# Sachin-A/TraceWeaver

Hardware: AMD Instinct MI355X
Metric: spans/sec reconstructed + assignment accuracy vs ground truth (higher is better)
Workload: dtype int64 timestamps, f64 scores; 1 GPU; media_microservices shape (6 services, E in {1,1,1,1,2,4}), 100000 requests/service x 16 replicas per GPU, concurrency 1.6, two-pass reconstruction, device mixture refit; spans_per_gpu=25600000, spans_total=25600000, parallelism=units sharded, 1 rank(s), backend none

## Files before the change

### traceweaver_amd/csrc/tw_engine.hip

```cpp
#include <algorithm>
#include <chrono>
#include <cmath>
#include <cstdio>
#include <cstdlib>
#include <cstring>
#include <functional>
#include <string>
#include <type_traits>
#include <vector>

#include <hip/hip_runtime.h>
#include <rocprim/rocprim.hpp>

#include "traceweaver_amd.h"
#include "tw_kernels.h"
#include "tw_fit.h"
#include "tw_eval.h"
#include "tw_skip.h"
#include "tw_load.h"
#include "tw_baselines.h"
#include "tw_stitch.h"
#include "tw_attr.h"
#include "tw_conf.h"
#include "tw_dist.h"
// ... 58 lines not shown
    hipEvent_t tile_ev[kMaxEp + 1] = {};
    hipStream_t cls_stream2[kMaxEp + 1] = {};
    hipEvent_t stretch_ev[kMaxEp + 1][kEnumStretches] = {}, stretch_done[kMaxEp + 1] = {};
    int enum_stretches = 1, stretch_min_tiles = 2048;
    int heavy_grid = 4096, select_grid = 0;
    int debug_lists = 0;
    int32_t first_lists[3][kMaxEp + 1] = {};
    hipEvent_t gate_ev = nullptr;
    int tile_gate = 0;
    int stage_min_tiles = 1024;
    int32_t *rank_in = nullptr, *rank_out = nullptr;
    bool class_params = false;
    int prio_min_e = 0, prio_high = 0;
    bool prio_any = false;
    int pipeline = 1;
    std::string err;
    int state = ST_EMPTY;
    int tile = kTile;
    int tile_threads = 2;
    int tile_single = 1;
    int tile_rank = 1;
    int block_params = 1;
    int tile_single_threads = 1;
    int coop = kCoop;
    std::vector<UnitDev> units;
    std::vector<TileDev> tiles;
    std::vector<int64_t> gs_off_h;
    std::vector<void*> allocs;
    void* arena = nullptr;
    size_t arena_cap = 0;
    bool arena_open = false;
    std::vector<std::pair<std::function<void(void*)>, size_t>> arena_req;
    Dev P{};
    int64_t n_ie = 0, n_gp = 0, n_slots = 0, n_gaps = 0;
    PairVI* agg_pair = nullptr;
    int32_t *agg_i32 = nullptr, *agg_i32b = nullptr;
    uint32_t *seg_in = nullptr, *seg_out = nullptr;
    int n_seg_out = 0;
    void* sort_tmp = nullptr;
    size_t sort_tmp_bytes = 0;
    double* mix_p_dev = nullptr;
    int32_t* mix_n_dev = nullptr;
    double* mix_c_dev = nullptr;
    double* gaps_sorted = nullptr;
    double* fit_models = nullptr;
    double* fit_uval = nullptr;
// ... 304 lines not shown
    const dim3 hb(std::min(e->coop, kHeavyThreads));
    const int pool = E > 4 ? 2048 : (E > 1 ? kPairPoolPerEp * E : 1);
    const size_t pool_bytes = sizeof(double) * (size_t)pool;
    const size_t lean_bytes = sizeof(double) * (size_t)(2 * kMaxEp * kNarrow + e->lean_pool), lean_bytes_w = sizeof(double) * (size_t)(2 * kMaxEp * 64 * kCandWords + e->lean_pool);
    const bool lean = E >= P.lean_min_e && !e->skip_mode;
    const int cap = P.heavy_in_off[E + 1] - P.heavy_in_off[E];
    auto grid_for = [&](int known, int most) { return std::max(std::min(((known >= 0 ? known : cap) + kWorkChunk - 1) / kWorkChunk, most), 1); };
    auto narrow = [&](int part, int g) {
        if (lean) hipLaunchKernelGGL((k_enumerate_lean<kNarrow>), dim3(g), hb, lean_bytes, st, P, pass, mode, part, e->lean_pool, E, E);
        else hipLaunchKernelGGL((k_enumerate_heavy<E, kNarrow>), dim3(g), hb, pool_bytes, st, P, pass, mode, part, pool);
    };
    auto wide = [&](int part, int g) {
        if (lean) hipLaunchKernelGGL((k_enumerate_lean<64 * kCandWords>), dim3(g), hb, lean_bytes_w, st, P, pass, mode, part, e->lean_pool, E, E);
        else hipLaunchKernelGGL((k_enumerate_heavy<E, 64 * kCandWords>), dim3(g), hb, pool_bytes, st, P, pass, mode, part, pool);
    };
    bool stretched = false;
    if (mode == 0 && pass == 1 && e->class_params) {
        const TileSet S = class_tiles(e, E);
        (void)sort_ends(e, S, st);
        launch_block_params(e, E, st);
    }
    if (mode == 0) {
        const bool single = E == 1 && e->tile_single != 0;
        const dim3 tile_block(e->tile >= 64 ? e->tile * (single ? e->tile_single_threads : e->tile_threads) : e->tile);
        int sub = 1;
        while (sub < e->tile_sub_max && nt * sub < 512 && (e->tile / (sub * 2)) * (sub * 2) == e->tile && e->tile / (sub * 2) >= 8) sub *= 2;
        const int ns = (!lean && !e->skip_mode && !(E >= 3 && E >= P.defer_min_e) && e->cls_stream2[E] != nullptr)
                           ? std::max(std::min(e->enum_stretches, nt / e->stretch_min_tiles), 1) : 1;
        stretched = ns > 1;
        for (int j = 0; j < ns; j++) {
            const int t0 = (int)((int64_t)nt * j / ns), t1 = (int)((int64_t)nt * (j + 1) / ns);
            const int32_t* ids = e->tile_ids + e->tile_cls_off[E] + t0;
            const bool sub_tile = e->tile == kTile && e->tile / sub == kSubTileSpans;
            if constexpr (E == 1) {
                if (single && sub_tile) hipLaunchKernelGGL((k_enumerate_tile<1, kSubTileSpans, true>), dim3((t1 - t0) * sub), tile_block, 0, st, P, pass, ids, t1 - t0, sub);
                else if (single) hipLaunchKernelGGL((k_enumerate_tile<1, kTile, true>), dim3((t1 - t0) * sub), tile_block, 0, st, P, pass, ids, t1 - t0, sub);
            }
            if (!single && sub_tile)
                hipLaunchKernelGGL((k_enumerate_tile<E, kSubTileSpans>), dim3((t1 - t0) * sub), tile_block, 0, st, P, pass, ids, t1 - t0, sub);
            else if (!single)
                hipLaunchKernelGGL((k_enumerate_tile<E>), dim3((t1 - t0) * sub), tile_block, 0, st, P, pass, ids, t1 - t0, sub);
            if (ns > 1) {
                hipLaunchKernelGGL(k_enum_snapshot, dim3(1), dim3(1), 0, st, P, E, j + 1);
                if (j + 1 < ns) {
                    hipStream_t s2 = e->cls_stream2[E];
                    (void)hipEventRecord(e->stretch_ev[E][j], st);
                    (void)hipStreamWaitEvent(s2, e->stretch_ev[E][j], 0);
                    hipLaunchKernelGGL((k_enumerate_heavy<E, kNarrow>), dim3(grid_for(-1, e->heavy_grid)), hb, pool_bytes, s2, P, pass, mode, (j + 1) << 8, pool);
                } else {
                    hipLaunchKernelGGL((k_enumerate_heavy<E, kNarrow>), dim3(grid_for(-1, e->heavy_grid)), hb, pool_bytes, st, P, pass, mode, (j + 1) << 8, pool);
                    (void)hipEventRecord(e->stretch_done[E], e->cls_stream2[E]);
                    (void)hipStreamWaitEvent(st, e->stretch_done[E], 0);
                }
            }
        }
        if (e->tile_gate > 0 && nt >= e->tile_gate) { (void)hipEventRecord(e->tile_ev[E], st); e->gate_ev = e->tile_ev[E]; }
    }
    if (n_narrow != 0 && !stretched) narrow(0, grid_for(n_narrow, e->heavy_grid));
    if (n_wide != 0) wide(0, grid_for(n_wide, 1024));
    if (mode == 0 && E >= 3 && E >= P.defer_min_e) { narrow(3, grid_for(-1, 4096)); if (n_wide != 0) wide(3, grid_for(-1, 1024)); }
    if (mode == 0 && E > 1) {
        const int nsplit = (pass == 2 && mode == 0) ? e->split_pass1[E] : -1;
        const int merge_grid = nsplit < 0 ? (cap >= (1 << 20) ? 1024 : 256) : std::max(std::min(nsplit, 1024), 8);
// ... 438 lines not shown
        if (unit_time_scale != nullptr) unit_time_scale[u] = U.tscale;
    }
    HIPCHK(hipMemcpyAsync(const_cast<UnitDev*>(P.units), e->units.data(), sizeof(UnitDev) * e->units.size(), hipMemcpyHostToDevice, e->stream));
    HIPCHK(hipStreamSynchronize(e->stream));
    e->state = ST_LOADED; e->pass1_done = false;
    drop_batch_order(e);
    for (int E = 0; E <= kMaxEp; E++) { e->wide_pass1[E] = -1; e->hard_pass1[E] = -1; e->split_pass1[E] = -1; }
    return TW_OK;
}

extern "C" {

int tw_create(int device_id, tw_engine** out) {
    if (out == nullptr) return TW_ERR_ARG;
    *out = nullptr;
    tw_engine* e = new tw_engine();
    e->device = device_id;
    e->tile = std::min(std::max(env_int("TW_TILE", kTile), 1), kTile);
    e->tile_threads = std::min(std::max(env_int("TW_TILE_THREADS", 2), 1), 4);
    e->tile_single = env_int("TW_TILE_SINGLE", 1);
    e->block_params = env_int("TW_BLOCK_PARAMS", 1);
    e->tile_rank = env_int("TW_TILE_RANK", 1) != 0 ? 1 : 0;
    e->tile_single_threads = std::min(std::max(env_int("TW_TILE_SINGLE_THREADS", 1), 1), 4);
    e->coop = std::min(std::max(env_int("TW_COOP_THREADS", kCoop), 1), kCoop);
    if (env_int("TW_SET_HW_QUEUES", 0) != 0) setenv("GPU_MAX_HW_QUEUES", "12", 0);
    hipError_t s = hipSetDevice(device_id);
    if (s == hipSuccess) s = hipStreamCreate(&e->stream);
    for (int i = 0; i < EV_COUNT && s == hipSuccess; i++) s = hipEventCreate(&e->ev[i]);
    for (int i = 0; i < SE_COUNT && s == hipSuccess; i++) s = hipEventCreate(&e->stage_ev[i]);
    const int prio_min_e = env_int("TW_PRIO_MIN_E", 0);
    int prio_least = 0, prio_greatest = 0;
    if (s == hipSuccess) s = hipDeviceGetStreamPriorityRange(&prio_least, &prio_greatest);
    e->prio_min_e = prio_min_e; e->prio_high = prio_greatest; e->prio_any = prio_greatest != prio_least;
    for (int i = 0; i <= kMaxEp + 1 && s == hipSuccess; i++) s = hipEventCreateWithFlags(&e->cls_ev[i], hipEventDisableTiming);
    if (s == hipSuccess) s = hipEventCreateWithFlags(&e->prep_ev, hipEventDisableTiming);
    for (int i = 0; i <= kMaxEp && s == hipSuccess; i++) {
        s = hipEventCreateWithFlags(&e->post_fork[i], hipEventDisableTiming);
        if (s == hipSuccess) s = hipEventCreateWithFlags(&e->tile_ev[i], hipEventDisableTiming);
        if (s == hipSuccess) s = hipEventCreateWithFlags(&e->post_done[i], hipEventDisableTiming);
        if (s == hipSuccess) s = hipEventCreateWithFlags(&e->stretch_done[i], hipEventDisableTiming);
        for (int j = 0; j < kEnumStretches && s == hipSuccess; j++) s = hipEventCreateWithFlags(&e->stretch_ev[i][j], hipEventDisableTiming);
        for (int j = 0; j < 3 && s == hipSuccess; j++) s = hipEventCreateWithFlags(&e->post_join[i][j], hipEventDisableTiming);
    }
    e->pipeline = env_int("TW_CLASS_PIPELINE", 1);
    e->sig_hash_bits = std::min(std::max(env_int("TW_SIG_HASH_BITS", 64), 1), 64);
    e->tile_gate = env_int("TW_TILE_GATE", 0);
// ... 2067 lines not shown
```

### traceweaver_amd/csrc/tw_tile.h

```cpp
#pragma once

namespace tw {

#ifndef TW_TILE_MAX
#define TW_TILE_MAX 256
#endif
constexpr int kTileMax = TW_TILE_MAX;
#ifndef TW_TILE_REPLAY_MAX
#define TW_TILE_REPLAY_MAX 256
#endif
constexpr int kTileReplayMax = TW_TILE_REPLAY_MAX;
#ifndef TW_TILE_RANK_DIRECT
#define TW_TILE_RANK_DIRECT 32
#endif
constexpr int kRankDirect = TW_TILE_RANK_DIRECT;
constexpr int kRankMinLong = (kRankDirect & ~3) + 4;
constexpr int kRankBuckets = 5;
static_assert(kRankDirect >= 24, "the maxima and counters of a segment's long spans lie in one byte per tuple slot");
__device__ __forceinline__ uint32_t score_key32(double v) {
    const unsigned long long u = (unsigned long long)__double_as_longlong(v + 0.0);
    return (uint32_t)(((u >> 63) ? ~u : (u | (1ull << 63))) >> 32);
}
__device__ __forceinline__ int pos_base(unsigned long long pk, int e) {
    int acc = 0;
    for (int f = 0; f < e; f++) acc += (int)((pk >> (8 * f)) & 255ull);
    return acc;
}
#ifndef TW_TILE_ITEMS
#define TW_TILE_ITEMS 768
#define TW_TILE_GRID 1024
#endif
constexpr int kSubTileSpans = kTile / 8;
template <int E, int SPANS = kTile>
struct TileCfg {
#ifdef TW_TILE_SMALL
    static constexpr int kSlice = 24, kItems = kMaxEp * 32, kGrid = kTileMax > 64 ? kTileMax : 64;
#else
    static constexpr int kSlice = SPANS < kTile ? 64 : (E <= 4 ? 192 : 160);
    static constexpr int kItems = SPANS < kTile ? kMaxEp * 32 : TW_TILE_ITEMS;
    static constexpr int kGrid = SPANS < kTile ? (kTileMax > 512 ? kTileMax : 512) : TW_TILE_GRID;
#endif
    static_assert(kItems >= kMaxEp * 32 && kGrid >= ((kTileMax + 3) & ~3) && kGrid % 4 == 0, "a single span must fit a segment");
};

__device__ __forceinline__ uint32_t div_small(uint32_t rest, uint32_t c) {
#ifdef TW_HOST_EMULATION
    const float rc = 1.0f / (float)c;
#else
    const float rc = __builtin_amdgcn_rcpf((float)c);
#endif
    return (uint32_t)(((float)rest + 0.5f) * rc);
}

__device__ __forceinline__ int fresh(int v) {
#ifndef TW_HOST_EMULATION
    asm volatile("" : "+v"(v));
#endif
    return v;
}

__device__ __forceinline__ double score_term_gap(const Scorer& S, int slot, long long gap) {
    const double x = (double)gap;
    if (S.pass == 1) {
        const double* g = S.gp + slot * 4;
        return term_gauss(g[0], g[3], g[2], x);
    }
    return score_term_mix_x(S, slot, x);
}

#ifdef TW_PROFILE_TILE
#ifndef TW_PROFILE_TILE_E
#define TW_PROFILE_TILE_E 4
#endif
#define TW_TILE_T0() long long _tp = wall_clock64(); const long long _tb = _tp; long long _ta[7] = {0, 0, 0, 0, 0, 0, 0}
#define TW_TILE_TICK(k) do { const long long _n = wall_clock64(); _ta[k] += _n - _tp; _tp = _n; } while (0)
#define TW_TILE_COUNT(k, v) do { if (E == TW_PROFILE_TILE_E && threadIdx.x == 0) atomicAdd((unsigned long long*)&P.prof[k], (unsigned long long)(v)); } while (0)
#define TW_TILE_FLUSH() do { if (E == TW_PROFILE_TILE_E && threadIdx.x == 0) { for (int _k = 0; _k < 7; _k++) atomicAdd((unsigned long long*)&P.prof[_k], (unsigned long long)_ta[_k]); \
    atomicAdd((unsigned long long*)&P.prof[7], (unsigned long long)(wall_clock64() - _tb)); atomicAdd((unsigned long long*)&P.prof[8], 1ull); } } while (0)
#else
#define TW_TILE_T0() do {} while (0)
#define TW_TILE_TICK(k) do {} while (0)
#define TW_TILE_COUNT(k, v) do {} while (0)
#define TW_TILE_FLUSH() do {} while (0)
#endif

#ifdef TW_HOST_EMULATION
#define TW_TILE_ATTR
#else
#define TW_TILE_ATTR __attribute__((amdgpu_waves_per_eu(SINGLE ? 8 : (E <= 4 ? 4 : 2))))
#endif
template <int E, int SPANS = kTile, bool SINGLE = false>
__global__ void __launch_bounds__(4 * kTile) TW_TILE_ATTR k_enumerate_tile(Dev P, int pass, const int32_t* tile_ids, int n_tiles_e, int sub_tiles) {
    static_assert(!SINGLE || E == 1, "the lean path is the one of a single endpoint");
    if (*P.err != 0) return;
    typedef TileCfg<E, SPANS> C;
    constexpr int SL = C::kSlice;
    const int vb = xcd_tile(blockIdx.x, n_tiles_e * sub_tiles);
    const int tile = tile_ids[vb / sub_tiles];
    const TileDev T = P.tiles[tile];
    const UnitDev& U = P.units[T.unit];
    const int t = threadIdx.x, nt = blockDim.x;
    const int sub_spans = P.tile_spans / sub_tiles, first = T.first + (vb % sub_tiles) * sub_spans;
    const int ns = min(sub_spans, min(P.tile_spans, U.n_in - T.first) - (vb % sub_tiles) * sub_spans);
    if (ns <= 0) return;
    __shared__ int32_t s_is[SPANS], s_ie[SPANS];
    __shared__ int32_t sl_st[E][SL], sl_en[E][SL];
    __shared__ int32_t s_A[E], s_B[E];
    __shared__ uint16_t s_lo[E][SPANS];
    __shared__ uint32_t s_cm[E][SPANS];
    __shared__ uint32_t s_bits[E][SPANS];
    __shared__ int32_t s_item0[SPANS + 1], s_grid0[SPANS + 1], s_leaves[SPANS];
    __shared__ uint8_t s_amb[SPANS];
    __shared__ unsigned long long s_cn[SPANS];
    __shared__ int32_t s_wtot[4 * kTile / 64][2];
    __shared__ double t_root[C::kItems], t_close[C::kItems];
    __shared__ uint16_t it_idx[C::kItems];
    __shared__ double g_sc[C::kGrid];
    __shared__ uint8_t g_span[C::kGrid];
    __shared__ uint32_t g_aux[C::kGrid / 4];
    __shared__ int32_t s_segend, s_anyamb;
    const bool live = t < ns;
    const int i = first + (live ? t : 0);
    const int64_t base = P.in_start[U.in_off + first];
    const int64_t in_start = P.in_start[U.in_off + i], in_end = P.in_end[U.in_off + i];
    const int64_t* os[E];
    const int64_t* oe[E];
#pragma unroll
    for (int e = 0; e < E; e++) { os[e] = P.out_start + U.ep_off[e]; oe[e] = P.out_end + U.ep_off[e]; }
    for (int x = t; x < E; x += nt) { s_A[x] = 0x7fffffff; s_B[x] = 0; }
    uint32_t dag_pm[E], dag_np[E], dag_pl[E];
    uint32_t ordered = 0;
#pragma unroll
    for (int e = 0; e < E; e++) {
        dag_pm[e] = U.pred_mask[e];
        dag_np[e] = U.npred[e];
        uint32_t pk = 0;
#pragma unroll
        for (int j = 0; j < E; j++) pk |= (j < (int)dag_np[e] ? ((uint32_t)U.pred_list[e][j] | ((uint32_t)U.pred_prim[e][j] << 3)) : 0u) << (4 * j);
        dag_pl[e] = pk;
        ordered |= dag_pm[e];
    }
    TW_TILE_T0();
    int32_t lo[E], hi[E];
    if (pass == 1) {
#pragma unroll
        for (int e = E - 1; e >= 0; e--) {
            const int n = (int)(U.ep_off[e + 1] - U.ep_off[e]);
            int64_t tmax = in_end;
#pragma unroll
            for (int f = e + 1; f < E; f++) {
                if (!((U.succ_mask[e] >> f) & 1)) continue;
                const int nf = (int)(U.ep_off[f + 1] - U.ep_off[f]);
                const int anchor = hi[f] >= 0 ? hi[f] : nf - 1;
                const int64_t st = os[f][anchor];
                if (st < tmax) tmax = st;
            }
            if (U.skip) {
                lo[e] = lower_bound_i64(os[e], n, in_start);
                hi[e] = upper_bound_i64(os[e], n, tmax) - 1;
            } else {
                lo[e] = bound_near<false>(os[e], n, in_start, i);
                hi[e] = bound_near<true>(os[e], n, tmax, lo[e]) - 1;
            }
        }
        if (live) {
#pragma unroll
            for (int e = 0; e < E; e++) { P.c_lo[ie_index(U, e, i)] = lo[e]; P.c_hi[ie_index(U, e, i)] = hi[e]; }
// ... 96 lines not shown
                if (any_order != 0) first_cands = 0;
            }
        }
        heavy_append<E>(P, live && !mine && !wide, narrow, hprod > kBigProduct, T.unit, i, hprod, U.skip ? 0 : first_cands, twins_any);
    }
    const bool some = mine && !empty && prod > 0;
    int nitem = 0;
    unsigned long long cnpack = 0;
    if (live) {
#pragma unroll
        for (int e = 0; e < E; e++) {
            const int rel = lo[e] - s_A[e], c = some ? __popcll((unsigned long long)cm[e]) : 0;
            s_lo[e][t] = (uint16_t)(some ? rel : 0);
            s_cm[e][t] = some ? cm[e] : 0u;
            if constexpr (!SINGLE) s_bits[e][t] = 0u;
            nitem += c;
            cnpack |= (unsigned long long)c << (8 * e);
        }
        s_is[t] = (int32_t)iso; s_ie[t] = (int32_t)ieo;
        s_amb[t] = 0;
        if constexpr (!SINGLE) { s_cn[t] = cnpack; s_leaves[t] = (some && !ordered) ? (int)prod : 0; }
    }
    {
        int a = live ? nitem : 0, b = (!SINGLE && live && some) ? (((int)prod + 3) & ~3) : 0;
        const int lane = t & 63, wv = t >> 6;
        for (int off = 1; off < 64; off <<= 1) {
            const int a2 = __shfl_up(a, off);
            if (lane >= off) a += a2;
            if constexpr (!SINGLE) { const int b2 = __shfl_up(b, off); if (lane >= off) b += b2; }
        }
        if (lane == 63 || t == nt - 1) { s_wtot[wv][0] = a; if constexpr (!SINGLE) s_wtot[wv][1] = b; }
        group_sync();
        for (int w = 0; w < wv; w++) { a += s_wtot[w][0]; if constexpr (!SINGLE) b += s_wtot[w][1]; }
        if (live) { s_item0[t + 1] = a; if constexpr (!SINGLE) s_grid0[t + 1] = b; }
        if (t == 0) { s_item0[0] = 0; if constexpr (!SINGLE) s_grid0[0] = 0; }
        group_sync();
    }
    TW_TILE_TICK(2);
    Scorer S;
    S.pass = pass;
    S.mix_n = P.mix_n + U.slot_off;
    S.mix_c = P.mix_c + (int64_t)U.slot_off * kMaxComp * 4;
    auto span_of = [&](const int32_t* pre, int first, int last, int x) -> int {
        int a = first, b = last - 1;
        while (a < b) { const int mid = (a + b + 1) >> 1; if (pre[mid] <= x) a = mid; else b = mid - 1; }
        return a;
    };
// ... 117 lines not shown
                }
                s_amb[tl] = 0;
            }
            if (here && s_mine[tl] && !s_amb[tl]) {
                const int i1 = first + tl;
                const int64_t g = U.in_off + i1;
                P.tk_n[g] = nitem1 < kTopK ? nitem1 : kTopK;
                P.leaves[g] = nitem1;
                if (pass == 1) P.leaves0[g] = nitem1;
                P.rep[g] = 0;
                if (pass == 1) {
                    P.c_bits[ie_index(U, 0, i1) * kCandWords] = (uint64_t)s_cm[0][tl];
                    for (int w = 1; w < kCandWords; w++) P.c_bits[ie_index(U, 0, i1) * kCandWords + w] = (uint64_t)(uint32_t)fresh(0);
                }
            }
            group_sync();
            TW_TILE_TICK(6);
            seg = send;
        }
        TW_TILE_FLUSH();
        const int te = fresh(t);
        heavy_append<E>(P, live && s_mine[te] != 0 && s_amb[te] != 0, true, false, T.unit, first + (live ? te : 0), 0, 0, false, te & 63);
        return;
    } else
    for (int seg = 0; seg < ns;) {
        constexpr int kLong = (C::kGrid - kRankMinLong) / kRankMinLong + 1;
        constexpr bool kRankFits = kLong * (kRankBuckets + 1) + 1 <= C::kGrid / 4 && C::kGrid * 4 <= C::kItems * 8 && C::kGrid <= 65536;
        static_assert(kRankBuckets == kTopK && C::kGrid <= C::kItems * 8, "a subset of slots per entry of the list; a rank per slot in t_root");
        uint32_t* const r_max = g_aux;
        int32_t* const r_cnt = reinterpret_cast<int32_t*>(g_aux + kLong * kRankBuckets);
        uint8_t* const g_rank = reinterpret_cast<uint8_t*>(t_root);
        uint16_t* const r_sub = reinterpret_cast<uint16_t*>(t_close);
        uint16_t* const r_all = r_sub + C::kGrid;
        const bool compact = kRankFits && P.tile_rank != 0;
        if (compact) for (int x = fresh(t); x < kLong * (kRankBuckets + 1) + 1; x += nt) g_aux[x] = 0u;
        if (t == 0) { s_segend = ns; s_anyamb = 0; }
        group_sync();
        if (live && t >= seg && (s_item0[t + 1] - s_item0[seg] > C::kItems || s_grid0[t + 1] - s_grid0[seg] > C::kGrid)) atomicMin(&s_segend, t);
        group_sync();
        const int send = s_segend;
        const int it0 = s_item0[seg], nIt = s_item0[send] - it0, g0 = s_grid0[seg], nG = s_grid0[send] - g0;
        TW_TILE_TICK(2);
        TW_TILE_COUNT(9, 1); TW_TILE_COUNT(10, nIt); TW_TILE_COUNT(11, nG);
        for (int k = t; k < nIt; k += nt) {
            const int s = span_of(s_item0, seg, send, it0 + k);
            int j = it0 + k - s_item0[s], es = 0;
            uint32_t m = 0;
            bool found = false;
#pragma unroll
            for (int e = 0; e < E; e++)
                if (!found) { m = s_cm[e][s]; const int c = __popcll((unsigned long long)m); if (j < c) { es = e; found = true; } else j -= c; }
            const int idx = (int)s_lo[es][s] + nth_set_bit((unsigned long long)m, j);
            int32_t st = 0, en = 0;
            bool is_root = false;
#pragma unroll
            for (int e = 0; e < E; e++) if (e == es) { st = sl_st[e][idx]; en = sl_en[e][idx]; is_root = dag_np[e] == 0; }
            S.gp = P.gparam + (U.gp_off + (int64_t)((first + s) / P.batch_size) * U.nslot) * 4;
            t_root[k] = is_root ? score_term_gap(S, slot_root(E, es), (long long)st - s_is[s]) : 0.0;
            t_close[k] = score_term_gap(S, slot_close(E, es), (long long)s_ie[s] - en);
            it_idx[k] = (uint16_t)idx;
        }
        group_sync();
        TW_TILE_TICK(3);
        for (int g = t; g < nG; g += nt) {
// ... 29 lines not shown
                    for (int j = 0; j < E; j++) {
                        if (j >= np) continue;
                        const uint32_t pj = (dag_pl[e] >> (4 * j)) & 15u;
                        if (!(pj & 8u)) continue;
                        const int p = (int)(pj & 7u);
                        int32_t pend = 0;
#pragma unroll
                        for (int q = 0; q < E; q++) if (q == p) pend = en[q];
                        sj += score_term_gap(S, slot_prim(E, p, e), (long long)st[e] - pend);
                    }
                    if (np == 0) sj += t_root[kx[e]];
                    if (e == last) sj += t_close[kx[e]];
                }
                if (ordered) {
                    atomicAdd(&s_leaves[s], 1);
                    if (pass == 1) {
#pragma unroll
                        for (int e = 0; e < E; e++) atomicOr(&s_bits[e][s], 1u << (ix[e] - (int)s_lo[e][s]));
                    }
                }
            }
            g_sc[g] = ok ? sj : dnan();
            g_span[g] = (uint8_t)s;
            if (compact && ok && s_grid0[s + 1] - s_grid0[s] > kRankDirect) {
                uint32_t* b = r_max + ((g - gi) / kRankMinLong) * kRankBuckets + gi % kRankBuckets;
                const uint32_t key = score_key32(sj);
                if (key > *(volatile uint32_t*)b) atomicMax(b, key);
            }
        }
        group_sync();
        TW_TILE_TICK(4);
        auto order_equal = [&](int s, const int32_t (&ia)[E], int hrel) -> int {
            int32_t kb[E], ib[E];
            decode(s, hrel, it0, kb, ib);
            int ord = 0;
            bool done = false;
#pragma unroll
            for (int e = 0; e < E; e++)
                if (!done && ia[e] != ib[e]) {
                    const int32_t a = sl_st[e][ia[e]], b = sl_st[e][ib[e]];
                    ord = b > a ? 1 : (b < a ? -1 : 0);
                    done = true;
                }
            return ord;
        };
        if (compact) {
            const int tr = fresh(t);
            for (int gb = 0; gb < nG; gb += nt) {
                const int g = gb + tr, lane = tr & 63;
                bool surv = false;
                int sub0 = 0;
                if (g < nG) {
                    const double my = g_sc[g];
                    const int s = g_span[g];
                    const int gs = s_grid0[s] - g0, ge = s_grid0[s + 1] - g0;
                    if (ge - gs > kRankDirect && my == my) {
                        const uint32_t* b = r_max + (gs / kRankMinLong) * kRankBuckets;
                        uint32_t lk = b[0];
#pragma unroll
                        for (int j = 1; j < kRankBuckets; j++) lk = b[j] < lk ? b[j] : lk;
                        surv = score_key32(my) >= lk;
                        sub0 = gs;
                    }
                }
                const int at = wave_append(&r_cnt[kLong], surv, lane);
                if (surv) r_all[at] = (uint16_t)g;
                unsigned long long todo = __ballot(surv);
                while (todo != 0ull) {
                    const int leader = __ffsll((long long)todo) - 1;
                    const int lead0 = __shfl(sub0, leader);
                    const bool with = surv && sub0 == lead0;
                    const unsigned long long m = __ballot(with);
                    int base = 0;
                    if (lane == leader) base = atomicAdd(&r_cnt[lead0 / kRankMinLong], __popcll(m));
                    base = __shfl(base, leader);
                    if (with) r_sub[lead0 + base + __popcll(m & ((1ull << lane) - 1ull))] = (uint16_t)g;
                    todo &= ~m;
                }
            }
        }
        for (int g = t; g < nG; g += nt) {
            const double my = g_sc[g];
            int rank = kTopK;
            const int s = g_span[g];
            const int gs = s_grid0[s] - g0, ge = s_grid0[s + 1] - g0;
            if (compact && ge - gs > kRankDirect) { g_rank[g] = (uint8_t)kTopK; continue; }
            if (my == my) {
                rank = 0;
                bool partner = false;
                int eq = 0;
                for (int h0 = gs; h0 < ge && rank < kTopK; h0 += 4) {
                    const double o0 = g_sc[h0], o1 = g_sc[h0 + 1], o2 = g_sc[h0 + 2], o3 = g_sc[h0 + 3];
                    rank += (o0 > my) + (o1 > my) + (o2 > my) + (o3 > my);
                    eq += (o0 == my) + (o1 == my) + (o2 == my) + (o3 == my);
                }
                if (eq > 1 && rank < kTopK) {
                    int32_t ka[E], ia[E];
                    decode(s, g - gs, it0, ka, ia);
                    for (int h = gs; h < ge; h++) {
                        if (h == g || !(g_sc[h] == my)) continue;
                        const int ord = order_equal(s, ia, h - gs);
                        if (ord > 0) rank++;
                        else if (ord == 0) partner = true;
                    }
                }
                if (partner && rank < kTopK) { s_amb[s] = 1; s_anyamb = 1; }
            }
            g_rank[g] = (uint8_t)(rank < kTopK ? rank : kTopK);
        }
        if (compact) {
            group_sync();
            const int nsv = r_cnt[kLong];
            for (int k = fresh(t); k < nsv; k += nt) {
                const int g = r_all[k];
                const double my = g_sc[g];
                const int s = g_span[g];
                const int gs = s_grid0[s] - g0;
                const int n = r_cnt[gs / kRankMinLong];
                const uint16_t* sub = r_sub + gs;
                int rank = 0, eq = 0;
                for (int h = 0; h < n && rank < kTopK; h++) {
                    const double o = g_sc[sub[h]];
                    rank += (o > my);
                    eq += (o == my);
                }
                bool partner = false;
                if (eq > 1 && rank < kTopK) {
                    int32_t ka[E], ia[E];
                    decode(s, g - gs, it0, ka, ia);
                    for (int h = 0; h < n; h++) {
                        const int hg = sub[h];
                        if (hg == g || !(g_sc[hg] == my)) continue;
                        const int ord = order_equal(s, ia, hg - gs);
                        if (ord > 0) rank++;
                        else if (ord == 0) partner = true;
                    }
                }
                if (partner && rank < kTopK) { s_amb[s] = 1; s_anyamb = 1; }
                g_rank[g] = (uint8_t)(rank < kTopK ? rank : kTopK);
            }
        }
        group_sync();
        TW_TILE_TICK(5);
        for (int g = t; g < nG; g += nt) {
            if (g_rank[g] >= kTopK) continue;
            const int s = g_span[g];
            if (s_amb[s]) continue;
            int32_t kx[E], ix[E];
            decode(s, g0 + g - s_grid0[s], it0, kx, ix);
            const int k = g_rank[g], si = first + s;
            P.tk_score[tks_index(U, k, si)] = g_sc[g];
#pragma unroll
            for (int e = 0; e < E; e++) P.tk_idx[tk_index(U, k, e, si)] = s_A[e] + ix[e];
        }
        if (s_anyamb != 0) group_sync();
        if (s_anyamb != 0 && live && t >= seg && t < send && mine && s_amb[t] && (t + 1) * (kTopK + 1) <= C::kItems && s_leaves[t] <= kTileReplayMax) {
            RegHeap RH;
            RH.clear(E);
            const unsigned long long pk = s_cn[t];
            auto start_of = [&](int e, int pos) -> int32_t { return sl_st[e][it_idx[s_item0[t] - it0 + pos_base(pk, e) + pos]]; };
            uint32_t real = 1;
#pragma unroll
            for (int e = 0; e < E; e++) real *= (uint32_t)((pk >> (8 * e)) & 255ull);
// ... 54 lines not shown
```

Measured before the change: 1.365 billion spans/s.

## Add specialized two-endpoint tile enumeration path with compact per-pair tables

Adds a PAIR specialization of the tile enumeration kernel for spans with exactly two endpoints. It uses smaller shared item and grid buffers, packs both candidate indices into 16 bits, and decodes the pair directly instead of using the generic E-way decode. This is meant to raise occupancy and cut decode overhead for the E=2 service class. The survivor-rank logic is factored into a shared helper, and threads in waves past the live span count skip range setup. The cost is another kernel instantiation and a duplicated code path whose correctness must match the generic one.

```diff
diff --git a/traceweaver_amd/csrc/tw_engine.hip b/traceweaver_amd/csrc/tw_engine.hip
--- a/traceweaver_amd/csrc/tw_engine.hip
+++ b/traceweaver_amd/csrc/tw_engine.hip
@@ -104,6 +104,8 @@
     int tile_rank = 1;
     int block_params = 1;
     int tile_single_threads = 1;
+    int tile_pair = 1;
+    int tile_pair_threads = 2;
     int coop = kCoop;
     std::vector<UnitDev> units;
     std::vector<TileDev> tiles;
@@ -454,7 +456,8 @@
     }
     if (mode == 0) {
         const bool single = E == 1 && e->tile_single != 0;
-        const dim3 tile_block(e->tile >= 64 ? e->tile * (single ? e->tile_single_threads : e->tile_threads) : e->tile);
+        const bool pair = E == 2 && e->tile_pair != 0;
+        const dim3 tile_block(e->tile >= 64 ? e->tile * (single ? e->tile_single_threads : (pair ? e->tile_pair_threads : e->tile_threads)) : e->tile);
         int sub = 1;
         while (sub < e->tile_sub_max && nt * sub < 512 && (e->tile / (sub * 2)) * (sub * 2) == e->tile && e->tile / (sub * 2) >= 8) sub *= 2;
         const int ns = (!lean && !e->skip_mode && !(E >= 3 && E >= P.defer_min_e) && e->cls_stream2[E] != nullptr)
@@ -468,9 +471,14 @@
                 if (single && sub_tile) hipLaunchKernelGGL((k_enumerate_tile<1, kSubTileSpans, true>), dim3((t1 - t0) * sub), tile_block, 0, st, P, pass, ids, t1 - t0, sub);
                 else if (single) hipLaunchKernelGGL((k_enumerate_tile<1, kTile, true>), dim3((t1 - t0) * sub), tile_block, 0, st, P, pass, ids, t1 - t0, sub);
             }
-            if (!single && sub_tile)
+            if constexpr (E == 2) {
+                if (pair && sub_tile) hipLaunchKernelGGL((k_enumerate_tile<2, kSubTileSpans, false, true>), dim3((t1 - t0) * sub), tile_block, 0, st, P, pass, ids, t1 - t0, sub);
+                else if (pair) hipLaunchKernelGGL((k_enumerate_tile<2, kTile, false, true>), dim3((t1 - t0) * sub), tile_block, 0, st, P, pass, ids, t1 - t0, sub);
+            }
+            if (single || pair) {}
+            else if (sub_tile)
                 hipLaunchKernelGGL((k_enumerate_tile<E, kSubTileSpans>), dim3((t1 - t0) * sub), tile_block, 0, st, P, pass, ids, t1 - t0, sub);
-            else if (!single)
+            else
                 hipLaunchKernelGGL((k_enumerate_tile<E>), dim3((t1 - t0) * sub), tile_block, 0, st, P, pass, ids, t1 - t0, sub);
             if (ns > 1) {
                 hipLaunchKernelGGL(k_enum_snapshot, dim3(1), dim3(1), 0, st, P, E, j + 1);
@@ -955,6 +963,8 @@
     e->block_params = env_int("TW_BLOCK_PARAMS", 1);
     e->tile_rank = env_int("TW_TILE_RANK", 1) != 0 ? 1 : 0;
     e->tile_single_threads = std::min(std::max(env_int("TW_TILE_SINGLE_THREADS", 1), 1), 4);
+    e->tile_pair = env_int("TW_TILE_PAIR", 1);
+    e->tile_pair_threads = std::min(std::max(env_int("TW_TILE_PAIR_THREADS", 2), 1), 2);
     e->coop = std::min(std::max(env_int("TW_COOP_THREADS", kCoop), 1), kCoop);
     if (env_int("TW_SET_HW_QUEUES", 0) != 0) setenv("GPU_MAX_HW_QUEUES", "12", 0);
     hipError_t s = hipSetDevice(device_id);
diff --git a/traceweaver_amd/csrc/tw_tile.h b/traceweaver_amd/csrc/tw_tile.h
--- a/traceweaver_amd/csrc/tw_tile.h
+++ b/traceweaver_amd/csrc/tw_tile.h
@@ -31,16 +31,20 @@
 #define TW_TILE_GRID 1024
 #endif
 constexpr int kSubTileSpans = kTile / 8;
-template <int E, int SPANS = kTile>
+#ifndef TW_TILE_PAIR_ITEMS
+#define TW_TILE_PAIR_ITEMS 512
+#define TW_TILE_PAIR_GRID 1024
+#endif
+template <int E, int SPANS = kTile, bool PAIR = false>
 struct TileCfg {
 #ifdef TW_TILE_SMALL
-    static constexpr int kSlice = 24, kItems = kMaxEp * 32, kGrid = kTileMax > 64 ? kTileMax : 64;
+    static constexpr int kSlice = 24, kItems = PAIR ? 2 * 32 : kMaxEp * 32, kGrid = kTileMax > 64 ? kTileMax : 64;
 #else
     static constexpr int kSlice = SPANS < kTile ? 64 : (E <= 4 ? 192 : 160);
-    static constexpr int kItems = SPANS < kTile ? kMaxEp * 32 : TW_TILE_ITEMS;
-    static constexpr int kGrid = SPANS < kTile ? (kTileMax > 512 ? kTileMax : 512) : TW_TILE_GRID;
-#endif
-    static_assert(kItems >= kMaxEp * 32 && kGrid >= ((kTileMax + 3) & ~3) && kGrid % 4 == 0, "a single span must fit a segment");
+    static constexpr int kItems = SPANS < kTile ? kMaxEp * 32 : (PAIR ? TW_TILE_PAIR_ITEMS : TW_TILE_ITEMS);
+    static constexpr int kGrid = SPANS < kTile ? (kTileMax > 512 ? kTileMax : 512) : (PAIR ? TW_TILE_PAIR_GRID : TW_TILE_GRID);
+#endif
+    static_assert(kItems >= (PAIR ? 2 : kMaxEp) * 32 && kGrid >= ((kTileMax + 3) & ~3) && kGrid % 4 == 0, "a single span must fit a segment");
 };
 
 __device__ __forceinline__ uint32_t div_small(uint32_t rest, uint32_t c) {
@@ -58,6 +62,93 @@
 #endif
     return v;
 }
+
+template <int GRID, int MINLONG>
+struct SurvivorRanks {
+    static constexpr int kLong = (GRID - MINLONG) / MINLONG + 1;
+    static constexpr int kAuxWords = kLong * (kRankBuckets + 1) + 1;
+    uint32_t* aux;
+    uint8_t* g_rank;
+    uint16_t* r_sub;
+    uint16_t* r_all;
+    const double* g_sc;
+    const uint8_t* g_span;
+    const int32_t* s_grid0;
+    int g0;
+    __device__ __forceinline__ uint32_t* r_max() const { return aux; }
+    __device__ __forceinline__ int32_t* r_cnt() const { return reinterpret_cast<int32_t*>(aux + kLong * kRankBuckets); }
+    __device__ __forceinline__ void clear(int t, int nt) const { for (int x = t; x < kAuxWords; x += nt) aux[x] = 0u; }
+    __device__ __forceinline__ void note(int g, int gi, double sj) const {
+        uint32_t* b = r_max() + ((g - gi) / MINLONG) * kRankBuckets + gi % kRankBuckets;
+        const uint32_t key = score_key32(sj);
+        if (key > *(volatile uint32_t*)b) atomicMax(b, key);
+    }
+    __device__ __forceinline__ void collect(int nG, int tr, int nt) const {
+        for (int gb = 0; gb < nG; gb += nt) {
+            const int g = gb + tr, lane = tr & 63;
+            bool surv = false;
+            int sub0 = 0;
+            if (g < nG) {
+                const double my = g_sc[g];
+                const int s = g_span[g];
+                const int gs = s_grid0[s] - g0, ge = s_grid0[s + 1] - g0;
+                if (ge - gs > kRankDirect && my == my) {
+                    const uint32_t* b = r_max() + (gs / MINLONG) * kRankBuckets;
+                    uint32_t lk = b[0];
+#pragma unroll
+                    for (int j = 1; j < kRankBuckets; j++) lk = b[j] < lk ? b[j] : lk;
+                    surv = score_key32(my) >= lk;
+                    sub0 = gs;
+                }
+            }
+            const int at = wave_append(&r_cnt()[kLong], surv, lane);
+            if (surv) r_all[at] = (uint16_t)g;
+            unsigned long long todo = __ballot(surv);
+            while (todo != 0ull) {
+                const int leader = __ffsll((long long)todo) - 1;
+                const int lead0 = __shfl(sub0, leader);
+                const bool with = surv && sub0 == lead0;
+                const unsigned long long m = __ballot(with);
+                int base = 0;
+                if (lane == leader) base = atomicAdd(&r_cnt()[lead0 / MINLONG], __popcll(m));
+                base = __shfl(base, leader);
+                if (with) r_sub[lead0 + base + __popcll(m & ((1ull << lane) - 1ull))] = (uint16_t)g;
+                todo &= ~m;
+            }
+        }
+    }
+    template <class MINE, class ORDER, class UNDECIDED>
+    __device__ __forceinline__ void rank(int t, int nt, const MINE& mine_of, const ORDER& order, const UNDECIDED& undecided) const {
+        const int nsv = r_cnt()[kLong];
+        for (int k = t; k < nsv; k += nt) {
+            const int g = r_all[k];
+            const double my = g_sc[g];
+            const int s = g_span[g];
+            const int gs = s_grid0[s] - g0;
+            const int n = r_cnt()[gs / MINLONG];
+            const uint16_t* sub = r_sub + gs;
+            int rank = 0, eq = 0;
+            for (int h = 0; h < n && rank < kTopK; h++) {
+                const double o = g_sc[sub[h]];
+                rank += (o > my);
+                eq += (o == my);
+            }
+            bool partner = false;
+            if (eq > 1 && rank < kTopK) {
+                const auto mine = mine_of(s, g - gs);
+                for (int h = 0; h < n; h++) {
+                    const int hg = sub[h];
+                    if (hg == g || !(g_sc[hg] == my)) continue;
+                    const int ord = order(s, mine, hg - gs);
+                    if (ord > 0) rank++;
+                    else if (ord == 0) partner = true;
+                }
+            }
+            if (partner && rank < kTopK) undecided(s);
+            g_rank[g] = (uint8_t)(rank < kTopK ? rank : kTopK);
+        }
+    }
+};
 
 __device__ __forceinline__ double score_term_gap(const Scorer& S, int slot, long long gap) {
     const double x = (double)gap;
@@ -87,13 +178,17 @@
 #ifdef TW_HOST_EMULATION
 #define TW_TILE_ATTR
 #else
-#define TW_TILE_ATTR __attribute__((amdgpu_waves_per_eu(SINGLE ? 8 : (E <= 4 ? 4 : 2))))
-#endif
-template <int E, int SPANS = kTile, bool SINGLE = false>
+#ifndef TW_TILE_PAIR_WAVES
+#define TW_TILE_PAIR_WAVES 4
+#endif
+#define TW_TILE_ATTR __attribute__((amdgpu_waves_per_eu(SINGLE ? 8 : (PAIR ? TW_TILE_PAIR_WAVES : (E <= 4 ? 4 : 2)))))
+#endif
+template <int E, int SPANS = kTile, bool SINGLE = false, bool PAIR = false>
 __global__ void __launch_bounds__(4 * kTile) TW_TILE_ATTR k_enumerate_tile(Dev P, int pass, const int32_t* tile_ids, int n_tiles_e, int sub_tiles) {
     static_assert(!SINGLE || E == 1, "the lean path is the one of a single endpoint");
+    static_assert(!PAIR || (E == 2 && !SINGLE), "the pair path is the one of two endpoints");
     if (*P.err != 0) return;
-    typedef TileCfg<E, SPANS> C;
+    typedef TileCfg<E, SPANS, PAIR> C;
     constexpr int SL = C::kSlice;
     const int vb = xcd_tile(blockIdx.x, n_tiles_e * sub_tiles);
     const int tile = tile_ids[vb / sub_tiles];
@@ -115,7 +210,7 @@
     __shared__ int32_t s_wtot[4 * kTile / 64][2];
     __shared__ double t_root[C::kItems], t_close[C::kItems];
     __shared__ uint16_t it_idx[C::kItems];
-    __shared__ double g_sc[C::kGrid];
+    __shared__ double g_sc[C::kGrid + (PAIR ? 4 : 0)];
     __shared__ uint8_t g_span[C::kGrid];
     __shared__ uint32_t g_aux[C::kGrid / 4];
     __shared__ int32_t s_segend, s_anyamb;
@@ -142,7 +237,10 @@
     }
     TW_TILE_T0();
     int32_t lo[E], hi[E];
-    if (pass == 1) {
+    if ((t & ~63) >= ns) {
+#pragma unroll
+        for (int e = 0; e < E; e++) { lo[e] = 0; hi[e] = -1; }
+    } else if (pass == 1) {
 #pragma unroll
         for (int e = E - 1; e >= 0; e--) {
             const int n = (int)(U.ep_off[e + 1] - U.ep_off[e]);
@@ -285,7 +383,7 @@
         if constexpr (!SINGLE) { s_cn[t] = cnpack; s_leaves[t] = (some && !ordered) ? (int)prod : 0; }
     }
     {
-        int a = live ? nitem : 0, b = (!SINGLE && live && some) ? (((int)prod + 3) & ~3) : 0;
+        int a = live ? nitem : 0, b = (!SINGLE && live && some) ? (PAIR ? (int)prod : (((int)prod + 3) & ~3)) : 0;
         const int lane = t & 63, wv = t >> 6;
         for (int off = 1; off < 64; off <<= 1) {
             const int a2 = __shfl_up(a, off);
@@ -449,24 +547,209 @@
         const int te = fresh(t);
         heavy_append<E>(P, live && s_mine[te] != 0 && s_amb[te] != 0, true, false, T.unit, first + (live ? te : 0), 0, 0, false, te & 63);
         return;
+    } else if constexpr (PAIR) {
+        static_assert(SL <= 256, "the slice positions of a tuple's two candidates lie in a byte each");
+        __shared__ uint8_t it_span[C::kItems];
+        __shared__ uint16_t g_ix[C::kGrid];
+        __shared__ uint8_t s_mine[SPANS];
+        if (live) s_mine[t] = mine ? 1 : 0;
+        typedef SurvivorRanks<C::kGrid, kRankDirect + 1> SR;
+        constexpr bool kRankFits = SR::kAuxWords <= C::kGrid / 4 && C::kGrid * 4 <= C::kItems * 8 && C::kGrid <= 65536;
+        static_assert(C::kGrid <= C::kItems * 8, "a rank per slot in t_root");
+        uint8_t* const g_rank = reinterpret_cast<uint8_t*>(t_root);
+        const bool compact = kRankFits && P.tile_rank != 0;
+        const bool prim = dag_np[1] != 0 && (dag_pl[1] & 8u) != 0;
+        for (int seg = 0; seg < ns;) {
+            if (compact) SR{g_aux, g_rank, nullptr, nullptr, g_sc, g_span, s_grid0, 0}.clear(t, nt);
+            if (t == 0) { s_segend = ns; s_anyamb = 0; }
+            group_sync();
+            if (live && t >= seg && (s_item0[t + 1] - s_item0[seg] > C::kItems || s_grid0[t + 1] - s_grid0[seg] > C::kGrid)) atomicMin(&s_segend, t);
+            group_sync();
+            const int send = s_segend;
+            const int it0 = s_item0[seg], nIt = s_item0[send] - it0, g0 = s_grid0[seg], nG = s_grid0[send] - g0;
+            const SR sr{g_aux, g_rank, reinterpret_cast<uint16_t*>(t_close), reinterpret_cast<uint16_t*>(t_close) + C::kGrid, g_sc, g_span, s_grid0, g0};
+            const int tq = fresh(t);
+            const bool here = tq < ns && tq >= seg && tq < send;
+            TW_TILE_TICK(2);
+            TW_TILE_COUNT(9, 1); TW_TILE_COUNT(10, nIt); TW_TILE_COUNT(11, nG);
+            if (here) {
+                int k = s_item0[tq] - it0;
+#pragma unroll
+                for (int e = 0; e < 2; e++) {
+                    const int rel = s_lo[e][tq];
+                    for (uint32_t m = s_cm[e][tq]; m != 0; m &= m - 1, k++) { it_span[k] = (uint8_t)tq; it_idx[k] = (uint16_t)((rel + __ffs((int)m) - 1) | (e << 15)); }
+                }
+                for (int g = s_grid0[tq] - g0, ge = s_grid0[tq + 1] - g0; g < ge; g++) g_span[g] = (uint8_t)tq;
+            }
+            group_sync();
+            for (int k = t; k < nIt; k += nt) {
+                const int s = it_span[k], e = it_idx[k] >> 15, idx = it_idx[k] & 0x7fff;
+                const int32_t st = sl_st[e][idx], en = sl_en[e][idx];
+                const bool is_root = (e == 0 ? dag_np[0] : dag_np[1]) == 0;
+                S.gp = P.gparam + (U.gp_off + (int64_t)((first + s) / P.batch_size) * U.nslot) * 4;
+                t_root[k] = is_root ? score_term_gap(S, slot_root(E, e), (long long)st - s_is[s]) : 0.0;
+                t_close[k] = score_term_gap(S, slot_close(E, e), (long long)s_ie[s] - en);
+            }
+            group_sync();
+            TW_TILE_TICK(3);
+            for (int g = t; g < nG; g += nt) {
+                const int s = g_span[g];
+                const int gi = g - (s_grid0[s] - g0);
+                const uint32_t pk = (uint32_t)s_cn[s], n0 = pk & 255u, n1 = (pk >> 8) & 255u;
+                const uint32_t k0 = n1 == 1 ? (uint32_t)gi : div_small((uint32_t)gi, n1), k1 = (uint32_t)gi - k0 * n1;
+                const int kx0 = s_item0[s] - it0 + (int)k0, kx1 = s_item0[s] - it0 + (int)(n0 + k1);
+                const int ix0 = it_idx[kx0], ix1 = it_idx[kx1] & 0x7fff;
+                const int32_t st0 = sl_st[0][ix0], en0 = sl_en[0][ix0], st1 = sl_st[1][ix1], en1 = sl_en[1][ix1];
+                const bool ok = !((dag_pm[1] & 1u) && en0 > st1);
+                double sj = 0.0;
+                if (ok) {
+                    const bool last1 = en1 > en0;
+                    if (dag_np[0] == 0) sj += t_root[kx0];
+                    if (!last1) sj += t_close[kx0];
+                    if (prim) {
+                        S.gp = P.gparam + (U.gp_off + (int64_t)((first + s) / P.batch_size) * U.nslot) * 4;
+                        sj += score_term_gap(S, slot_prim(E, 0, 1), (long long)st1 - en0);
+                    }
+                    if (dag_np[1] == 0) sj += t_root[kx1];
+                    if (last1) sj += t_close[kx1];
+                    if (ordered) {
+                        atomicAdd(&s_leaves[s], 1);
+                        if (pass == 1) { atomicOr(&s_bits[0][s], 1u << (ix0 - (int)s_lo[0][s])); atomicOr(&s_bits[1][s], 1u << (ix1 - (int)s_lo[1][s])); }
+                    }
+                }
+                g_sc[g] = ok ? sj : dnan();
+                g_ix[g] = (uint16_t)(ix0 | (ix1 << 8));
+                if (compact && ok && s_grid0[s + 1] - s_grid0[s] > kRankDirect) sr.note(g, gi, sj);
+            }
+            group_sync();
+            TW_TILE_TICK(4);
+            auto order_equal = [&](uint32_t a, uint32_t b) -> int {
+                const int e = (a & 255u) != (b & 255u) ? 0 : 1;
+                const int32_t sa = sl_st[e][(a >> (8 * e)) & 255u], sb = sl_st[e][(b >> (8 * e)) & 255u];
+                return sb > sa ? 1 : (sb < sa ? -1 : 0);
+            };
+            if (compact) sr.collect(nG, t, nt);
+            for (int g = t; g < nG; g += nt) {
+                const double my = g_sc[g];
+                int rank = kTopK;
+                const int s = g_span[g];
+                const int gs = s_grid0[s] - g0, ge = s_grid0[s + 1] - g0;
+                if (compact && ge - gs > kRankDirect) { g_rank[g] = (uint8_t)kTopK; continue; }
+                if (my == my) {
+                    rank = 0;
+                    bool partner = false;
+                    int eq = 0;
+                    for (int h0 = gs; h0 < ge && rank < kTopK; h0 += 4) {
+                        const double o0 = g_sc[h0], o1 = g_sc[h0 + 1], o2 = g_sc[h0 + 2], o3 = g_sc[h0 + 3];
+                        const bool in1 = h0 + 1 < ge, in2 = h0 + 2 < ge, in3 = h0 + 3 < ge;
+                        rank += (o0 > my) + (in1 && o1 > my) + (in2 && o2 > my) + (in3 && o3 > my);
+                        eq += (o0 == my) + (in1 && o1 == my) + (in2 && o2 == my) + (in3 && o3 == my);
+                    }
+                    if (eq > 1 && rank < kTopK) {
+                        const uint32_t mine_ix = g_ix[g];
+                        for (int h = gs; h < ge; h++) {
+                            if (h == g || !(g_sc[h] == my)) continue;
+                            const int ord = order_equal(mine_ix, g_ix[h]);
+                            if (ord > 0) rank++;
+                            else if (ord == 0) partner = true;
+                        }
+                    }
+                    if (partner && rank < kTopK) { s_amb[s] = 1; s_anyamb = 1; }
+                }
+                g_rank[g] = (uint8_t)(rank < kTopK ? rank : kTopK);
+            }
+            if (compact) {
+                group_sync();
+                sr.rank(t, nt,
+                        [&](int s, int gi) -> uint32_t { return g_ix[s_grid0[s] - g0 + gi]; },
+                        [&](int s, uint32_t mine_ix, int hrel) { return order_equal(mine_ix, g_ix[s_grid0[s] - g0 + hrel]); },
+                        [&](int s) { s_amb[s] = 1; s_anyamb = 1; });
+            }
+            group_sync();
+            TW_TILE_TICK(5);
+            for (int g = t; g < nG; g += nt) {
+                if (g_rank[g] >= kTopK) continue;
+                const int s = g_span[g];
+                if (s_amb[s]) continue;
+                const int k = g_rank[g], si = first + s;
+                const uint32_t ix = g_ix[g];
+                P.tk_score[tks_index(U, k, si)] = g_sc[g];
+                P.tk_idx[tk_index(U, k, 0, si)] = s_A[0] + (int)(ix & 255u);
+                P.tk_idx[tk_index(U, k, 1, si)] = s_A[1] + (int)(ix >> 8);
+            }
+            if (s_anyamb != 0) group_sync();
+            const int tl = fresh(t);
+            const bool mine_here = tl < ns && tl >= seg && tl < send && s_mine[tl] != 0;
+            const int th = tl < SPANS / 2 ? tl : tl - SPANS / 2;
+            const bool replay = s_anyamb != 0 && mine_here && s_amb[tl] && (th + 1) * (kTopK + 1) <= C::kItems && (tl + 1) * (kTopK + 1) <= C::kGrid && s_leaves[tl] <= kTileReplayMax;
+            if (replay) {
+                const int ks = s_item0[tl] - it0;
+                const int c0 = (int)((uint32_t)s_cn[tl] & 255u);
+                auto start_of = [&](int e, int pos) -> int32_t { return sl_st[e][it_idx[ks + (e != 0 ? c0 : 0) + pos] & 0x7fff]; };
+                RegHeap RH;
+                RH.clear(E);
+                const int gs = s_grid0[tl] - g0, nT = s_grid0[tl + 1] - s_grid0[tl];
+                const uint32_t n1 = ((uint32_t)s_cn[tl] >> 8) & 255u;
+                uint32_t k0 = 0, k1 = 0;
+                for (int gi = 0; gi < nT; gi++) {
+                    const double sc = g_sc[gs + gi];
+                    const unsigned long long x = (unsigned long long)(k0 | (k1 << 8));
+                    if (++k1 == n1) { k1 = 0; k0++; }
+                    if (!(sc == sc) || RH.below_root(sc)) continue;
+                    RH.push(sc, x, start_of);
+                }
+                double* hs = (tl < SPANS / 2 ? t_root : t_close) + th * (kTopK + 1);
+                uint16_t* hx = g_ix + tl * (kTopK + 1);
+#pragma unroll
+                for (int k = 0; k < kTopK; k++) { hs[k] = RH.s[k]; hx[k] = (uint16_t)RH.x[k]; }
+                py_sort_desc(hs, hx, RH.n, [&](double sa, unsigned long long xa, double sb, unsigned long long xb) { return RH.lt(sa, xa, sb, xb, start_of); });
+                const int si = first + tl;
+                for (int k = 0; k < RH.n; k++) {
+                    P.tk_score[tks_index(U, k, si)] = hs[k];
+                    P.tk_idx[tk_index(U, k, 0, si)] = s_A[0] + (int)it_idx[ks + (int)(hx[k] & 255u)];
+                    P.tk_idx[tk_index(U, k, 1, si)] = s_A[1] + (int)(it_idx[ks + c0 + (int)(hx[k] >> 8)] & 0x7fff);
+                }
+                s_amb[tl] = 0;
+            }
+            if (mine_here && !s_amb[tl]) {
+                const int i = first + tl;
+                const int64_t g = U.in_off + i;
+                const int leaves = s_leaves[tl];
+                P.tk_n[g] = leaves < kTopK ? leaves : kTopK;
+                P.leaves[g] = leaves;
+                if (pass == 1) P.leaves0[g] = leaves;
+                P.rep[g] = 0;
+                if (pass == 1) {
+#pragma unroll
+                    for (int e = 0; e < 2; e++) {
+                        P.c_bits[ie_index(U, e, i) * kCandWords] = (uint64_t)(ordered ? s_bits[e][tl] : s_cm[e][tl]);
+                        for (int w = 1; w < kCandWords; w++) P.c_bits[ie_index(U, e, i) * kCandWords + w] = 0;
+                    }
+                }
+            }
+            group_sync();
+            TW_TILE_TICK(6);
+            seg = send;
+        }
+        TW_TILE_FLUSH();
+        const int te = fresh(t);
+        heavy_append<E>(P, te < ns && s_mine[te] != 0 && s_amb[te] != 0, true, false, T.unit, first + (te < ns ? te : 0), 0, 0, false, te & 63);
+        return;
     } else
     for (int seg = 0; seg < ns;) {
-        constexpr int kLong = (C::kGrid - kRankMinLong) / kRankMinLong + 1;
-        constexpr bool kRankFits = kLong * (kRankBuckets + 1) + 1 <= C::kGrid / 4 && C::kGrid * 4 <= C::kItems * 8 && C::kGrid <= 65536;
+        typedef SurvivorRanks<C::kGrid, kRankMinLong> SR;
+        constexpr bool kRankFits = SR::kAuxWords <= C::kGrid / 4 && C::kGrid * 4 <= C::kItems * 8 && C::kGrid <= 65536;
         static_assert(kRankBuckets == kTopK && C::kGrid <= C::kItems * 8, "a subset of slots per entry of the list; a rank per slot in t_root");
-        uint32_t* const r_max = g_aux;
-        int32_t* const r_cnt = reinterpret_cast<int32_t*>(g_aux + kLong * kRankBuckets);
         uint8_t* const g_rank = reinterpret_cast<uint8_t*>(t_root);
-        uint16_t* const r_sub = reinterpret_cast<uint16_t*>(t_close);
-        uint16_t* const r_all = r_sub + C::kGrid;
         const bool compact = kRankFits && P.tile_rank != 0;
-        if (compact) for (int x = fresh(t); x < kLong * (kRankBuckets + 1) + 1; x += nt) g_aux[x] = 0u;
+        if (compact) SR{g_aux, g_rank, nullptr, nullptr, g_sc, g_span, s_grid0, 0}.clear(fresh(t), nt);
         if (t == 0) { s_segend = ns; s_anyamb = 0; }
         group_sync();
         if (live && t >= seg && (s_item0[t + 1] - s_item0[seg] > C::kItems || s_grid0[t + 1] - s_grid0[seg] > C::kGrid)) atomicMin(&s_segend, t);
         group_sync();
         const int send = s_segend;
         const int it0 = s_item0[seg], nIt = s_item0[send] - it0, g0 = s_grid0[seg], nG = s_grid0[send] - g0;
+        const SR sr{g_aux, g_rank, reinterpret_cast<uint16_t*>(t_close), reinterpret_cast<uint16_t*>(t_close) + C::kGrid, g_sc, g_span, s_grid0, g0};
         TW_TILE_TICK(2);
         TW_TILE_COUNT(9, 1); TW_TILE_COUNT(10, nIt); TW_TILE_COUNT(11, nG);
         for (int k = t; k < nIt; k += nt) {
@@ -542,11 +825,7 @@
             }
             g_sc[g] = ok ? sj : dnan();
             g_span[g] = (uint8_t)s;
-            if (compact && ok && s_grid0[s + 1] - s_grid0[s] > kRankDirect) {
-                uint32_t* b = r_max + ((g - gi) / kRankMinLong) * kRankBuckets + gi % kRankBuckets;
-                const uint32_t key = score_key32(sj);
-                if (key > *(volatile uint32_t*)b) atomicMax(b, key);
-            }
+            if (compact && ok && s_grid0[s + 1] - s_grid0[s] > kRankDirect) sr.note(g, gi, sj);
         }
         group_sync();
         TW_TILE_TICK(4);
@@ -564,41 +843,7 @@
                 }
             return ord;
         };
-        if (compact) {
-            const int tr = fresh(t);
-            for (int gb = 0; gb < nG; gb += nt) {
-                const int g = gb + tr, lane = tr & 63;
-                bool surv = false;
-                int sub0 = 0;
-                if (g < nG) {
-                    const double my = g_sc[g];
-                    const int s = g_span[g];
-                    const int gs = s_grid0[s] - g0, ge = s_grid0[s + 1] - g0;
-                    if (ge - gs > kRankDirect && my == my) {
-                        const uint32_t* b = r_max + (gs / kRankMinLong) * kRankBuckets;
-                        uint32_t lk = b[0];
-#pragma unroll
-                        for (int j = 1; j < kRankBuckets; j++) lk = b[j] < lk ? b[j] : lk;
-                        surv = score_key32(my) >= lk;
-                        sub0 = gs;
-                    }
-                }
-                const int at = wave_append(&r_cnt[kLong], surv, lane);
-                if (surv) r_all[at] = (uint16_t)g;
-                unsigned long long todo = __ballot(surv);
-                while (todo != 0ull) {
-                    const int leader = __ffsll((long long)todo) - 1;
-                    const int lead0 = __shfl(sub0, leader);
-                    const bool with = surv && sub0 == lead0;
-                    const unsigned long long m = __ballot(with);
-                    int base = 0;
-                    if (lane == leader) base = atomicAdd(&r_cnt[lead0 / kRankMinLong], __popcll(m));
-                    base = __shfl(base, leader);
-                    if (with) r_sub[lead0 + base + __popcll(m & ((1ull << lane) - 1ull))] = (uint16_t)g;
-                    todo &= ~m;
-                }
-            }
-        }
+        if (compact) sr.collect(nG, fresh(t), nt);
         for (int g = t; g < nG; g += nt) {
             const double my = g_sc[g];
             int rank = kTopK;
@@ -630,35 +875,11 @@
         }
         if (compact) {
             group_sync();
-            const int nsv = r_cnt[kLong];
-            for (int k = fresh(t); k < nsv; k += nt) {
-                const int g = r_all[k];
-                const double my = g_sc[g];
-                const int s = g_span[g];
-                const int gs = s_grid0[s] - g0;
-                const int n = r_cnt[gs / kRankMinLong];
-                const uint16_t* sub = r_sub + gs;
-                int rank = 0, eq = 0;
-                for (int h = 0; h < n && rank < kTopK; h++) {
-                    const double o = g_sc[sub[h]];
-                    rank += (o > my);
-                    eq += (o == my);
-                }
-                bool partner = false;
-                if (eq > 1 && rank < kTopK) {
-                    int32_t ka[E], ia[E];
-                    decode(s, g - gs, it0, ka, ia);
-                    for (int h = 0; h < n; h++) {
-                        const int hg = sub[h];
-                        if (hg == g || !(g_sc[hg] == my)) continue;
-                        const int ord = order_equal(s, ia, hg - gs);
-                        if (ord > 0) rank++;
-                        else if (ord == 0) partner = true;
-                    }
-                }
-                if (partner && rank < kTopK) { s_amb[s] = 1; s_anyamb = 1; }
-                g_rank[g] = (uint8_t)(rank < kTopK ? rank : kTopK);
-            }
+            struct Mine { int32_t ia[E]; };
+            sr.rank(fresh(t), nt,
+                    [&](int s, int gi) { Mine m; int32_t ka[E]; decode(s, gi, it0, ka, m.ia); return m; },
+                    [&](int s, const Mine& m, int hrel) { return order_equal(s, m.ia, hrel); },
+                    [&](int s) { s_amb[s] = 1; s_anyamb = 1; });
         }
         group_sync();
         TW_TILE_TICK(5);
```

After: 1.382 billion spans/s (median of 6 runs). 1.3% higher.
